# ibrohimmn1994/GPU-implementation-of-signle-and-block-Lanczos

Measured on AMD Instinct MI355X. Metric: block-Lanczos iters/sec + SpMM achieved HBM GB/s vs peak, n=10M nnz=1e8 b=16, higher is better.
Workload: dtype f64; 1 GPU; C3 block Lanczos b=16 fp64, banded-random symmetric CSR n=10000000 per GPU, nnz~10/row, halfwidth 4096; config=C3, n_total=10000000, n_per_gpu=10000000, nnz_per_gpu=100000182, b=16, parallelism=single

## Files before the change

### gpu-implementation-of-signle-and-block-lanczos_amd/__init__.py

```python
from __future__ import annotations

import ctypes
import os
from dataclasses import dataclass
from typing import NamedTuple, Optional

import numpy as np

PKG_DIR = os.path.dirname(os.path.abspath(__file__))
LIB_DIR = os.path.join(PKG_DIR, "lib")
HIP_LIB = os.environ.get("LZ_HIP_LIB") or os.path.join(LIB_DIR, "liblz_hip.so")
HOST_LIB = os.path.join(LIB_DIR, "liblz_host.so")

LZ_F64, LZ_F32 = 0, 1
LZ_ROW_MAJOR, LZ_COL_MAJOR = 0, 1
(LZ_K_SEG768, LZ_K_SEG1536, LZ_K_SEG1024, LZ_K_FNZ, LZ_K_BUF, LZ_K_LDS, LZ_K_ANY_B, LZ_K_CM_DIRECT,
 LZ_K_SPMV) = range(1, 10)
LZ_K_WIN, LZ_K_YCM, LZ_K_EPI, LZ_K_AX3, LZ_K_DOT = 0x100, 0x200, 0x400, 0x800, 0x1000
LZ_K_AX4 = 0x2000
LZ_K_GRAM16, LZ_K_GRAM32F, LZ_K_GRAM_GEN, LZ_K_TSMM16, LZ_K_TSMM32F, LZ_K_TSMM_GEN = range(1, 7)
LZ_K_PGRAM16, LZ_K_PGRAM_GEN, LZ_K_PAPPLY16, LZ_K_PAPPLY_GEN = range(7, 11)
PANEL_GROUP_16, PANEL_GROUP_GEN = 16, 4
PANEL_MAX_BLOCKS = 64
LZ_K_PCOMP16, LZ_K_PCOMP_GEN = 11, 12
PANEL_MAX_KEEP = 16
TRANSPOSE_SHORT, TRANSPOSE_LDS, TRANSPOSE_SCAN_BLOCK = 16, 4096, 2048
CG_THREADS, CG_ROWS_128, CG_GRID_CAP, CG_CHECK_EVERY = 256, 32, 2048, 8
CG_MET, CG_SPENT, CG_NOT_PD = 0, 1, 2
BCG_THREADS, BCG_ROWS_16, BCG_ROWS_32, BCG_ROWS_GEN, BCG_GRID_CAP, BCG_MAX_B = 256, 64, 128, 16, 1024, 32
LZ_K_BCG16, LZ_K_BCG32F, LZ_K_BCG_GEN = 13, 14, 15
BCG_NONE, BCG_CONVERGED, BCG_SPENT, BCG_RANK, BCG_NOT_PD = 0, 1, 2, 3, 4


def bcg_guard(b: int, eps: float) -> float:
    return max(1e-10, 64.0 * b * eps)


# ... 7 lines not shown

_hip = None
_host = None

HIP_SYMBOLS = [
    ("lz_init", _c_int, [_c_int, ctypes.POINTER(_c_vp)]),
    ("lz_finalize", _c_int, [_c_vp]),
    ("lz_set_stream", _c_int, [_c_vp, _c_vp]),
    ("lz_set_final_state", _c_int, [_c_vp, _c_int]),
    ("lz_last_error", ctypes.c_char_p, []),
    ("lz_version", ctypes.c_char_p, []),
    ("lz_device_ok", _c_int, [_c_int]),
    ("lz_device_error", _c_int, [_c_vp, ctypes.POINTER(_c_int)]),
    ("lz_debug_poison_lds", _c_int, [_c_vp, ctypes.c_uint32]),
    ("lz_debug_set_device_error", _c_int, [_c_vp, _c_int]),
    ("lz_debug_fail_next_setup", _c_int, [_c_vp, _c_int]),
    ("lz_prof_enable", _c_int, [_c_vp, _c_int]),
    ("lz_prof_enable_mask", _c_int, [_c_vp, ctypes.c_uint]),
    ("lz_prof_read", _c_int, [_c_vp, _c_int, ctypes.POINTER(_c_dbl), ctypes.POINTER(_c_int)]),
    ("lz_csr_spmm", _c_int, [_c_vp, _c_i64, _c_i64, _c_i64, _c_vp, _c_vp, _c_vp, _c_int, _c_int,
                             _c_vp, _c_i64, _c_int, _c_vp, _c_i64]),
    ("lz_to_row_major", _c_int, [_c_vp, _c_i64, _c_int, _c_int, _c_vp, _c_i64, _c_vp]),
    ("lz_to_col_major", _c_int, [_c_vp, _c_i64, _c_int, _c_int, _c_vp, _c_vp, _c_i64]),
    ("lz_csr_spmv", _c_int, [_c_vp, _c_i64, _c_i64, _c_i64, _c_vp, _c_vp, _c_vp, _c_int, _c_vp, _c_vp]),
    ("lz_gram", _c_int, [_c_vp, _c_i64, _c_int, _c_int, _c_vp, _c_i64, _c_vp]),
    ("lz_sym_cross_gram", _c_int, [_c_vp, _c_i64, _c_int, _c_int, _c_vp, _c_vp, _c_i64, _c_vp]),
    ("lz_tsmm", _c_int, [_c_vp, _c_i64, _c_int, _c_int, _c_dbl, _c_dbl, _c_vp, _c_vp, _c_vp, _c_i64]),
    ("lz_sqrtm_pair", _c_int, [_c_vp, _c_int, _c_int, _c_vp, _c_vp, _c_vp, _c_vp]),
    ("lz_copy_row", _c_int, [_c_vp, _c_int, _c_int, _c_vp, _c_i64, _c_int, _c_i64, _c_vp, _c_i64]),
    ("lz_block_lanczos", _c_int, [_c_vp, _c_i64, _c_i64, _c_vp, _c_vp, _c_vp, _c_int, _c_int, _c_int,
                                  _c_i64, _c_vp, _c_vp, _c_vp, _c_vp, _c_vp, _c_vp, _c_vp]),
    ("lz_block_lanczos_unfused", _c_int, [_c_vp, _c_i64, _c_i64, _c_vp, _c_vp, _c_vp, _c_int, _c_int,
                                          _c_int, _c_i64, _c_vp, _c_vp, _c_vp, _c_vp, _c_vp, _c_vp, _c_vp]),
    ("lz_panel_gram", _c_int, [_c_vp, _c_i64, _c_int, _c_int, _c_int, _c_vp, _c_i64, _c_vp, _c_vp]),
    ("lz_panel_apply", _c_int, [_c_vp, _c_i64, _c_int, _c_int, _c_int, _c_dbl, _c_dbl, _c_vp, _c_i64, _c_vp, _c_vp]),
    ("lz_block_lanczos_reorth", _c_int, [_c_vp, _c_i64, _c_i64, _c_vp, _c_vp, _c_vp, _c_int, _c_int, _c_int,
                                         _c_i64, _c_vp, _c_vp, _c_vp, _c_vp, _c_vp, _c_i64, _c_vp, _c_int]),
    ("lz_panel_compress", _c_int, [_c_vp, _c_i64, _c_int, _c_int, _c_int, _c_int, _c_vp, _c_i64, _c_vp]),
    ("lz_block_lanczos_reorth_resume", _c_int, [_c_vp, _c_i64, _c_i64, _c_vp, _c_vp, _c_vp, _c_int, _c_int, _c_int,
                                                _c_int, _c_i64, _c_vp, _c_vp, _c_vp, _c_vp, _c_vp, _c_i64, _c_vp,
                                                _c_int]),
    ("lz_csr_spmm_axpby", _c_int, [_c_vp, _c_i64, _c_i64, _c_vp, _c_vp, _c_vp, _c_int, _c_int, _c_dbl, _c_vp,
                                   _c_dbl, _c_dbl, _c_vp, _c_vp]),
    ("lz_cheb_apply", _c_int, [_c_vp, _c_i64, _c_i64, _c_vp, _c_vp, _c_vp, _c_int, _c_int, _c_vp, _c_vp, _c_vp,
                               _c_vp]),
    ("lz_col_dots", _c_int, [_c_vp, _c_i64, _c_int, _c_int, _c_vp, _c_vp, _c_vp]),
    ("lz_csr_spmm_axpby_dots", _c_int, [_c_vp, _c_i64, _c_i64, _c_vp, _c_vp, _c_vp, _c_int, _c_int, _c_dbl, _c_vp,
                                        _c_dbl, _c_dbl, _c_vp, _c_vp, _c_vp]),
    ("lz_cheb_moments", _c_int, [_c_vp, _c_i64, _c_i64, _c_vp, _c_vp, _c_vp, _c_int, _c_int, _c_dbl, _c_dbl, _c_int,
                                 _c_vp, _c_vp, _c_vp]),
    ("lz_cg_update", _c_int, [_c_vp, _c_i64, _c_int, _c_int, _c_vp, _c_vp, _c_vp, _c_vp, _c_vp, _c_vp, _c_vp]),
    ("lz_cg_solve", _c_int, [_c_vp, _c_i64, _c_i64, _c_vp, _c_vp, _c_vp, _c_int, _c_int, _c_dbl, _c_vp, _c_vp, _c_vp,
                             _c_vp, _c_vp, _c_vp, _c_vp, _c_vp, _c_vp]),
    ("lz_bcg_update", _c_int, [_c_vp, _c_i64, _c_int, _c_int, _c_vp, _c_vp, _c_vp, _c_vp, _c_vp, _c_vp, _c_vp]),
    ("lz_bcg_direction", _c_int, [_c_vp, _c_i64, _c_int, _c_int, _c_vp, _c_vp, _c_vp, _c_vp]),
    ("lz_bcg_solve", _c_int, [_c_vp, _c_i64, _c_i64, _c_vp, _c_vp, _c_vp, _c_int, _c_int, _c_dbl, _c_vp, _c_vp, _c_vp,
                              _c_vp, _c_vp, _c_vp, _c_vp, _c_vp, _c_vp]),
    ("lz_block_lanczos_reorth_cheb", _c_int, [_c_vp, _c_i64, _c_i64, _c_vp, _c_vp, _c_vp, _c_int, _c_int, _c_int,
                                              _c_i64, _c_vp, _c_vp, _c_vp, _c_vp, _c_vp, _c_i64, _c_vp, _c_int,
                                              _c_vp, _c_vp]),
    ("lz_block_lanczos_reorth_resume_cheb", _c_int, [_c_vp, _c_i64, _c_i64, _c_vp, _c_vp, _c_vp, _c_int, _c_int,
                                                     _c_int, _c_int, _c_i64, _c_vp, _c_vp, _c_vp, _c_vp, _c_vp,
                                                     _c_i64, _c_vp, _c_int, _c_vp, _c_vp]),
    ("lz_csr_spmm_axpby4", _c_int, [_c_vp, _c_i64, _c_i64, _c_vp, _c_vp, _c_vp, _c_int, _c_int, _c_dbl, _c_vp,
                                    _c_dbl, _c_dbl, _c_vp, _c_dbl, _c_vp, _c_vp]),
    ("lz_cheb_series_apply", _c_int, [_c_vp, _c_i64, _c_i64, _c_vp, _c_vp, _c_vp, _c_int, _c_int, _c_int, _c_dbl,
# ... 493 lines not shown
        raise LanczosError("bad CSR file")
    rp = np.empty(n.value + 1, np.int64)
    col = np.empty(nnz.value, np.int32)
    val = np.empty(nnz.value, np.float64 if dt.value == 0 else np.float32)
    if L.lzh_csr_read(path.encode(), _p(rp), _p(col), _p(val)):
        raise LanczosError("CSR read failed")
    return CsrHost(n.value, rp, col, val)


def _torch():
    import torch
    return torch


def _ld(t) -> int:
    if t.shape[1] > 1 and t.stride(1) != 1:
        raise LanczosError("inner dimension must be contiguous")
    return t.stride(0) if t.shape[0] > 1 else t.shape[1]


def _ptr(t) -> Optional[int]:
    return None if t is None else t.data_ptr()


def _dt(t) -> int:
    torch = _torch()
    if t.dtype == torch.float64:
        return LZ_F64
    if t.dtype == torch.float32:
        return LZ_F32
    raise LanczosError(f"unsupported dtype {t.dtype}")


@dataclass
class CsrDevice:
    n: int
    n_cols: int
    row_ptr: "object"
    col: "object"
    val: "object"

    @property
    def nnz(self) -> int:
        return int(self.col.numel())

    @property
    def dtype(self) -> int:
        return _dt(self.val)

    @staticmethod
    def from_host(A: CsrHost, device="cuda", n_cols: Optional[int] = None) -> "CsrDevice":
        torch = _torch()
        return CsrDevice(A.n, A.n if n_cols is None else n_cols,
                         torch.from_numpy(A.row_ptr).to(device),
                         torch.from_numpy(A.col).to(device),
                         torch.from_numpy(A.val).to(device))

    def transpose(self, handle: "Handle") -> "CsrDevice":
        torch = _torch()
        dev = self.val.device
        t_rp = torch.empty(self.n_cols + 1, dtype=torch.int64, device=dev)
        t_col = torch.empty(self.nnz, dtype=torch.int32, device=dev)
        t_val = torch.empty(self.nnz, dtype=self.val.dtype, device=dev)
        _check(handle.L.lz_csr_transpose(handle.ptr, self.n, self.n_cols, self.nnz, _ptr(self.row_ptr), _ptr(self.col),
                                         _ptr(self.val), self.dtype, _ptr(t_rp), _ptr(t_col), _ptr(t_val)),
               "lz_csr_transpose")
        return CsrDevice(self.n_cols, self.n, t_rp, t_col, t_val)


class _ReorthOp(NamedTuple):
    name: str
    head: tuple
    tail: tuple
    filt: object


def _f64(t) -> np.ndarray:
# ... 407 lines not shown
        n, b = W.shape
        _check(self.L.lz_gram(self.ptr, n, b, _dt(W), _ptr(W), W.stride(0), _ptr(R)), "lz_gram")
        return R

    def mm_tt2(self, W, Q, R):
        n, b = W.shape
        if Q.shape != W.shape or (n > 1 and Q.stride(0) != W.stride(0)):
            raise LanczosError("mm_tt2: W and Q must have the same shape and row stride (one ld for both)")
        _check(self.L.lz_sym_cross_gram(self.ptr, n, b, _dt(W), _ptr(W), _ptr(Q), W.stride(0), _ptr(R)),
               "lz_sym_cross_gram")
        return R

    def mm_ts(self, beta: float, alpha: float, Q, S, W):
        n, b = Q.shape
        if W.shape != Q.shape or (n > 1 and Q.stride(0) != W.stride(0)):
            raise LanczosError("mm_ts: Q and W must have the same shape and row stride (one ld for both)")
        _check(self.L.lz_tsmm(self.ptr, n, b, _dt(Q), beta, alpha, _ptr(Q), _ptr(S), _ptr(W), W.stride(0)),
               "lz_tsmm")
        return W

    def sqrtm(self, G, beta, beta_inv, eigval=None):
        b = G.shape[0]
        _check(self.L.lz_sqrtm_pair(self.ptr, b, _dt(G), _ptr(G), _ptr(beta), _ptr(beta_inv), _ptr(eigval)),
               "lz_sqrtm_pair")

    def copy_row_to_vector(self, lc: int, start: int, Q, q, layout: int = LZ_ROW_MAJOR):
        b = Q.shape[1] if layout == LZ_ROW_MAJOR else Q.shape[0]
        _check(self.L.lz_copy_row(self.ptr, b, _dt(Q), _ptr(Q), Q.stride(0), layout, lc, _ptr(q), start),
               "lz_copy_row")

    def block_lanczos_blas(self, A: CsrDevice, B, m: int, lc: int, q, alpha, beta, Q0, Q1, W,
                           fused: bool = True):
        n, b = B.shape
        fn = self.L.lz_block_lanczos if fused else self.L.lz_block_lanczos_unfused
        _check(fn(self.ptr, n, A.nnz, _ptr(A.row_ptr), _ptr(A.col), _ptr(A.val), A.dtype, b, m, lc,
                  _ptr(B), _ptr(q), _ptr(alpha), _ptr(beta), _ptr(Q0), _ptr(Q1), _ptr(W)),
               "lz_block_lanczos")

    @staticmethod
    def _panel(V, vstride: int, n: int, b: int, k: int):
        if V.dim() != 1 or not V.is_contiguous() or V.numel() < (k - 1) * vstride + n * b:
            raise LanczosError("a basis panel is a flat contiguous tensor of at least (k-1)*vstride + n*b elements")

    def panel_gram(self, V, vstride: int, k: int, W, C):
        n, b = W.shape
        self._panel(V, vstride, n, b, max(k, 1))
        if not W.is_contiguous() or not C.is_contiguous() or C.numel() < k * b * b or C.dtype != W.dtype \
                or V.dtype != W.dtype:
            raise LanczosError("panel_gram: W (n, b) and C (k, b, b) contiguous, one dtype")
        _check(self.L.lz_panel_gram(self.ptr, n, b, k, _dt(W), _ptr(V), vstride, _ptr(W), _ptr(C)), "lz_panel_gram")
        return C

    def panel_apply(self, beta: float, alpha: float, V, vstride: int, k: int, S, W):
        n, b = W.shape
        self._panel(V, vstride, n, b, max(k, 1))
        if not W.is_contiguous() or not S.is_contiguous() or S.numel() < k * b * b or S.dtype != W.dtype \
                or V.dtype != W.dtype:
            raise LanczosError("panel_apply: W (n, b) and S (k, b, b) contiguous, one dtype")
        _check(self.L.lz_panel_apply(self.ptr, n, b, k, _dt(W), beta, alpha, _ptr(V), vstride, _ptr(S), _ptr(W)),
               "lz_panel_apply")
        return W

    def block_lanczos_reorth(self, A: CsrDevice, B, m: int, lc: int, q, alpha, beta, V, vstride: int, W,
                             passes: int = 2, filt=None, work=None, normal=None, series=None):
        n, b = B.shape
        self._panel(V, vstride, n, b, max(m, 1))
        op = self._reorth_op("block_lanczos_reorth", A, n, b, W, filt, work, normal, series)
        _check(getattr(self.L, op.name)(self.ptr, *op.head, b, m, lc, _ptr(B), _ptr(q), _ptr(alpha), _ptr(beta),
                                        _ptr(V), vstride, _ptr(W), passes, *op.tail), op.name)

# ... 464 lines not shown
```

### gpu-implementation-of-signle-and-block-lanczos_amd/csrc/lz_api.hip

```cpp
#include <cmath>
#include <cstdarg>
#include <cstdlib>
#include <cstring>
#include <algorithm>
#include <utility>
#include <vector>

#include <type_traits>
#include "lz_comm.hpp"
#include "lz_common.hpp"
#include "lz_internal.hpp"
#include "lz_kernels.hpp"

namespace lz {

static thread_local char g_err[1024] = "";

int prof_begin(lz_handle *h, int cls)
{
    if (!h->prof || !((h->prof_mask >> cls) & 1u) || h->ev_used + 2 > h->ev_cap) return -1;
    const int idx = h->ev_used;
    if (hipEventRecord(h->ev_pool[idx], h->stream) != hipSuccess) return -1;
    h->ev_class[idx / 2] = cls;
    h->ev_used += 2;
// ... 1561 lines not shown
                             int64_t lc, const void *B, void *q, void *alpha, void *beta, void *Q0,
                             void *Q1, void *W)
{
    LZ_HANDLE_CHECK(h);
    LZ_TRY(block_args(n, nnz, rp, col, val, b, m, lc, B, q, alpha, beta, Q0, Q1, W));
    return by_dtype(dtype, [&](auto t) {
        using T = decltype(t);
        return block_lanczos_unfused<T>(h, n, nnz, rp, col, (const T *)val, b, m, lc, (const T *)B, (T *)q,
                                        (T *)alpha, (T *)beta, (T *)Q0, (T *)Q1, (T *)W);
    });
}

int lz_block_lanczos(lz_handle *h, int64_t n, int64_t nnz, const int64_t *rp, const int32_t *col,
                     const void *val, lz_dtype dtype, int b, int m, int64_t lc, const void *B,
                     void *q, void *alpha, void *beta, void *Q0, void *Q1, void *W)
{
    LZ_HANDLE_CHECK(h);
    LZ_TRY(block_args(n, nnz, rp, col, val, b, m, lc, B, q, alpha, beta, Q0, Q1, W));
    return by_dtype(dtype, [&](auto t) -> int {
        using T = decltype(t);
        const T *v = (const T *)val, *Bt = (const T *)B;
        T *qt = (T *)q, *at = (T *)alpha, *bt = (T *)beta, *q0 = (T *)Q0, *q1 = (T *)Q1, *w = (T *)W;
        if constexpr (std::is_same<T, double>::value) {
            if (b == 16) {
                LZ_TRY(solve_begin(h));
                LZ_TRY(block_lanczos_fused16(h, n, nnz, rp, col, v, m, lc, Bt, qt, at, bt, q0, q1, w));
                return solve_status(h);
            }
        }
        return block_lanczos_sep<T>(h, n, nnz, rp, col, v, b, m, lc, Bt, qt, at, bt, q0, q1, w);
    });
}

static int panel_args(int64_t n, int b, int k, lz_dtype dtype, const void *V, int64_t vstride)
{
    LZ_ARG_CHECK(dtype == LZ_F64 || dtype == LZ_F32, "dtype");
    LZ_ARG_CHECK(n >= 1, "n >= 1");
    LZ_ARG_CHECK(b >= 1 && b <= 32, "a basis panel supports 1 <= b <= 32");
    LZ_ARG_CHECK(k >= 1 && k <= kPanelMaxK, "a basis panel holds 1 <= k <= 64 blocks");
    LZ_ARG_CHECK(V != nullptr, "V is NULL");
    LZ_ARG_CHECK(vstride >= n * b, "vstride >= n*b");
    const int64_t per16 = dtype == LZ_F64 ? 2 : 4;
    LZ_ARG_CHECK(vstride % per16 == 0 && reinterpret_cast<uintptr_t>(V) % 16 == 0,
                 "V and vstride must be multiples of 16 bytes");
    return LZ_OK;
}

int lz_panel_gram(lz_handle *h, int64_t n, int b, int k, lz_dtype dtype, const void *V, int64_t vstride,
                  const void *W, void *C)
{
    LZ_HANDLE_CHECK(h);
    LZ_TRY(panel_args(n, b, k, dtype, V, vstride));
    LZ_ARG_CHECK(W && C, "W/C NULL");
    return by_dtype(dtype, [&](auto t) {
        using T = decltype(t);
        return panel_gram<T>(h, n, b, k, (const T *)V, vstride, (const T *)W, (T *)C);
    });
}

int lz_panel_apply(lz_handle *h, int64_t n, int b, int k, lz_dtype dtype, double beta, double alpha, const void *V,
                   int64_t vstride, const void *S, void *W)
{
    LZ_HANDLE_CHECK(h);
    LZ_TRY(panel_args(n, b, k, dtype, V, vstride));
    LZ_ARG_CHECK(S && W, "S/W NULL");
    {
// ... 794 lines not shown
```

### gpu-implementation-of-signle-and-block-lanczos_amd/csrc/lz_common.hpp

```cpp
#pragma once
#include <hip/hip_runtime.h>

#include <cstdint>
#include <cstdio>
#include <string>

#include "lz_hip.h"

namespace lz {

class Comm;

void set_error(const char *fmt, ...);

#define LZ_HIP_TRY(expr)                                                          \
    do {                                                                          \
        hipError_t e_ = (expr);                                                   \
        if (e_ != hipSuccess) {                                                   \
            ::lz::set_error("%s:%d %s -> %s", __FILE__, __LINE__, #expr,          \
                            hipGetErrorString(e_));                               \
            return LZ_E_HIP;                                                      \
        }                                                                         \
    } while (0)

// ... 24 lines not shown
constexpr int kWave = 64;
constexpr int kMaxPartials = 2048;
constexpr int kMaxB = 64;
constexpr int kMaxSolveB = 32;
constexpr size_t kScratchDoubles = 8 * kMaxB * kMaxB;
constexpr size_t kPartials2Doubles = 256 * kMaxB * kMaxB + 4096 * 256;

__host__ __device__ inline int64_t ceil_div(int64_t a, int64_t b) { return (a + b - 1) / b; }

}

struct lz_handle {
    int device = 0;
    hipStream_t stream = nullptr;
    hipStream_t side = nullptr;
    hipEvent_t ev_fork = nullptr, ev_join = nullptr;
    int n_cu = 256;
    int grid_cap = 0;
    double *partials = nullptr;
    size_t partials_cap = 0;
    double *partials2 = nullptr;
    double *scratch = nullptr;
    int *err_flag = nullptr;
    lz::Comm *comm = nullptr;
    int nranks = 1, rank = 0;
    hipStream_t xstream = nullptr;
    hipEvent_t ev_cx = nullptr, ev_xd = nullptr;
    hipEvent_t ev_bd = nullptr;
    int64_t last_split[2] = {-1, -1};
    int last_wf = 0, last_wf_pre = 0;
    int last_kernel[2] = {0, 0};
    int final_state = 1;
    int dbg_setup_fail = 0;
    void *c16buf = nullptr;
    size_t c16_cap = 0;
    int32_t *fnz_colf = nullptr, *fnz_trow = nullptr;
    int64_t fnz_key[4] = {0, 0, 0, 0};
    bool fnz_ok = false;
    void *wf_deps = nullptr;
    int *wf_flags = nullptr;
    size_t wf_deps_cap = 0, wf_flags_cap = 0;
    void *ybuf = nullptr;
    size_t ybuf_cap = 0;
    void *coef = nullptr;
    size_t coef_cap = 0;
    void *tr_ws = nullptr;
    size_t tr_cap = 0;
    void *halo = nullptr;
    uint64_t *pairs = nullptr;
    int *longq = nullptr;
    size_t longq_cap = 0;
    int longq_parity = 0;
    hipStream_t lstream = nullptr;
    hipEvent_t ev_lfork = nullptr, ev_ljoin = nullptr;
    hipStream_t pf_sg = nullptr, pf_sp = nullptr;
    hipEvent_t ev_pff = nullptr, ev_pfg = nullptr, ev_pfp = nullptr;
    int *pf_ctl = nullptr;
    int pf_key = -1;
    int pf_band = 0;
    int64_t pf_band_key[3] = {0, 0, -1};
    size_t pairs_cap = 0;
    void *cm_buf = nullptr;
    size_t cm_cap = 0;
    double *dots_ws = nullptr;
    size_t dots_cap = 0;
    void *cg_ws = nullptr;
// ... 82 lines not shown
```

### gpu-implementation-of-signle-and-block-lanczos_amd/csrc/lz_internal.hpp

```cpp
#pragma once
#include "lz_common.hpp"

namespace lz {

template <typename T>
int spmm_rm(lz_handle *h, int64_t n, int64_t nnz, const int64_t *rp, const int32_t *col, const T *val, int b,
            const T *X, int64_t ldx, int64_t nx, T *Y, int64_t ldy,
            bool ycm = false);
template <typename T>
struct SpmmTerms {
    T a;
    const T *X;
    T c, d;
    const T *Z;
    T e = T(0);
    const T *U = nullptr;
    bool four = false;
};
template <typename T>
int spmm_terms(lz_handle *h, int64_t n, int64_t nnz, const int64_t *rp, const int32_t *col, const T *val, int b,
               SpmmTerms<T> t, T *Y, double *dots = nullptr, bool fused = true, bool fused_dot = true);
template <typename T>
int spmm_cm(lz_handle *h, int64_t n, int64_t nnz, const int64_t *rp, const int32_t *col, const T *val, int b,
            const T *X, int64_t ldx, int64_t nx, T *Y, int64_t ldy);
// ... 97 lines not shown

struct WfPlan {
    bool ok = false;
    int hback = 0, hfwd = 0;
    int nc = 12, tr = 192;
    int var = 0;
    const int16_t *col16 = nullptr;
    int64_t xoff = 0;
    bool planned = false;
};
bool wf_first_gram(int64_t n, int64_t nnz);
int wf_plan16(lz_handle *h, int64_t n, int64_t nnz, const int64_t *rp, const int32_t *col, WfPlan *pl,
              int64_t nx = -1, int64_t xoff = 0);
int wf_reset16(lz_handle *h, int64_t n, const WfPlan &pl);
int wf_step16(lz_handle *h, int64_t n, const int64_t *rp, const int32_t *col, const int16_t *col16,
              const double *val, const uint64_t *pairs, const WfPlan &pl, const double *Yj, const double *Vprev,
              const double *Vj, double *Vout, const double *binv, const double *P1, const double *P2,
              const double *Vg, double *Yo, int epoch, int *nparts, int64_t nx = -1, int64_t p1a = 0,
              int64_t p1b = -1, double *part = nullptr, const int64_t *q = nullptr, double *Vsave = nullptr,
              bool qo = false);
struct WfSlabs {
    static constexpr int kMax = 6;
    const double *p[kMax] = {};
    int g[kMax] = {};
    int k = 0;
    void add(const double *ptr, int nslab)
    {
        p[k] = ptr;
        g[k] = nslab;
        ++k;
    }
};
int wf_fold16(lz_handle *h, const WfSlabs &sl, double *out);
int alpha_wf16(lz_handle *h, const double *part, int P, const double *binv, const double *P1, double *alpha,
               double *P2, const double *V, int64_t lc, int64_t n, double *qrow);

int fused_e32(lz_handle *h, int64_t n, const float *Y, const float *Wj, const float *Wprev, float *Wn,
              const float *binv, const float *P1, int64_t lc, float *qrow, int *nparts);
int fused_u32(lz_handle *h, int64_t n, float *Wn, const float *Wj, const float *P2, int *nparts);
int fused_el32(lz_handle *h, int64_t n, const float *Wj, const float *U, int *nparts);
int fused_ub32(lz_handle *h, int64_t n, const float *U, const float *Wj, const float *binv, const float *P2,
               float *Wn, int *nparts, float *Qa = nullptr,
               float *Qb = nullptr);
int alpha_b2(lz_handle *h, const double *part, int P, const float *binv, float *alpha, float *P2, const float *Wj,
             int64_t lc, int64_t n, float *qrow);
int m_b2(lz_handle *h, const double *part, int P, const float *binv, float *M);
bool spmm_b2_ok(int64_t n, int64_t nnz, int64_t nx);
int fold_slabs_g(lz_handle *h, const double *part, int64_t P, int bb, int G);
int spmm_rm_b2(lz_handle *h, int64_t n, int64_t nnz, const int64_t *rp, const int32_t *col, const float *val,
               const float *X, int64_t nx, float *Y, const float *Wp, const float *Mm, int plan_slot = -1,
               int *slot_out = nullptr, int cap = 768);
int spmm_b2_stage(lz_handle *h, int64_t n, const int64_t *rp, int *cap);
int spmm_b2_plan(lz_handle *h, int64_t n, const int64_t *rp, int cap, int *slot);
template <typename T>
int fused_e_sep(lz_handle *h, int64_t n, int b, const T *Y, const T *Wj, const T *Wprev, T *Wn, const T *binv,
                const T *P1, int64_t lc, T *qrow, int *nparts);
template <typename T>
int fused_u_sep(lz_handle *h, int64_t n, int b, T *Wn, const T *Wj, const T *P2, int *nparts);
template <typename T>
int fused_u_swap_sep(lz_handle *h, int64_t n, int b, T *Wn, T *Xown, const T *P2, int *nparts);

template <typename T>
int vector_lanczos_dev(lz_handle *h, int64_t n, int64_t nnz, const int64_t *rp, const int32_t *col,
                       const T *val, int m, int64_t lc, const T *b, T *q, T *alpha, T *beta, T *q0,
                       T *q1, T *w);

// ... 2 lines not shown
```

### include/lz_hip.h

```cpp
#ifndef LZ_HIP_H
#define LZ_HIP_H
#include <stddef.h>
#include <stdint.h>

#ifdef __cplusplus
extern "C" {
#endif

typedef enum { LZ_F64 = 0, LZ_F32 = 1 } lz_dtype;
typedef enum { LZ_ROW_MAJOR = 0, LZ_COL_MAJOR = 1 } lz_layout;

enum {
    LZ_OK = 0,
    LZ_E_ARG = -1,
    LZ_E_HIP = -2,
    LZ_E_COMM = -3,
    LZ_E_STATE = -4,
    LZ_E_DEVICE = -5
};

typedef struct lz_handle lz_handle;

int lz_init(int device, lz_handle **h);
int lz_finalize(lz_handle *h);
// ... 13 lines not shown
int lz_prof_enable_mask(lz_handle *h, unsigned class_mask);
int lz_prof_read(lz_handle *h, int kernel_class, double *ms_total, int *count);

int lz_csr_spmm(lz_handle *h, int64_t n_rows, int64_t n_cols, int64_t nnz,
                const int64_t *row_ptr, const int32_t *col, const void *val, lz_dtype dtype,
                int b, const void *X, int64_t ldx, lz_layout layout, void *Y, int64_t ldy);

int lz_to_row_major(lz_handle *h, int64_t rows, int b, lz_dtype dtype, const void *X, int64_t ldx, void *Y);

int lz_to_col_major(lz_handle *h, int64_t rows, int b, lz_dtype dtype, const void *X, void *Y, int64_t ldy);

int lz_csr_spmv(lz_handle *h, int64_t n_rows, int64_t n_cols, int64_t nnz,
                const int64_t *row_ptr, const int32_t *col, const void *val, lz_dtype dtype,
                const void *x, void *y);

int lz_gram(lz_handle *h, int64_t n, int b, lz_dtype dtype, const void *W, int64_t ld, void *R);

int lz_sym_cross_gram(lz_handle *h, int64_t n, int b, lz_dtype dtype, const void *W,
                      const void *Q, int64_t ld, void *R);

int lz_tsmm(lz_handle *h, int64_t n, int b, lz_dtype dtype, double beta, double alpha,
            const void *Q, const void *S, void *W, int64_t ld);

int lz_sqrtm_pair(lz_handle *h, int b, lz_dtype dtype, const void *G, void *beta,
                  void *beta_inv, void *eigval);

int lz_copy_row(lz_handle *h, int b, lz_dtype dtype, const void *Q, int64_t ld, lz_layout layout,
                int64_t lc, void *q, int64_t start);

int lz_block_lanczos(lz_handle *h, int64_t n, int64_t nnz, const int64_t *row_ptr,
                     const int32_t *col, const void *val, lz_dtype dtype, int b, int m,
                     int64_t lc, const void *B, void *q, void *alpha, void *beta, void *Q0,
                     void *Q1, void *W);

int lz_block_lanczos_unfused(lz_handle *h, int64_t n, int64_t nnz, const int64_t *row_ptr,
                             const int32_t *col, const void *val, lz_dtype dtype, int b, int m,
                             int64_t lc, const void *B, void *q, void *alpha, void *beta,
                             void *Q0, void *Q1, void *W);

int lz_panel_gram(lz_handle *h, int64_t n, int b, int k, lz_dtype dtype, const void *V, int64_t vstride,
                  const void *W, void *C);
int lz_panel_apply(lz_handle *h, int64_t n, int b, int k, lz_dtype dtype, double beta, double alpha,
                   const void *V, int64_t vstride, const void *S, void *W);
#define LZ_PANEL_MAX_KEEP 16
int lz_panel_compress(lz_handle *h, int64_t n, int b, int k, int r, lz_dtype dtype, void *V, int64_t vstride,
                      const void *Z);

int lz_block_lanczos_reorth(lz_handle *h, int64_t n, int64_t nnz, const int64_t *row_ptr,
                            const int32_t *col, const void *val, lz_dtype dtype, int b, int m,
                            int64_t lc, const void *B, void *q, void *alpha, void *beta, void *V,
                            int64_t vstride, void *W, int passes);

int lz_block_lanczos_reorth_resume(lz_handle *h, int64_t n, int64_t nnz, const int64_t *row_ptr,
                                   const int32_t *col, const void *val, lz_dtype dtype, int b, int r, int m,
                                   int64_t lc, const void *sigma, void *q, void *alpha, void *beta, void *V,
                                   int64_t vstride, void *W, int passes);

int lz_csr_spmm_axpby(lz_handle *h, int64_t n, int64_t nnz, const int64_t *row_ptr, const int32_t *col,
                      const void *val, lz_dtype dtype, int b, double a, const void *X, double c, double d,
                      const void *Z, void *Y);

typedef struct {
    int degree;
    double lo, hi, ref;
} lz_cheb;
int lz_cheb_apply(lz_handle *h, int64_t n, int64_t nnz, const int64_t *row_ptr, const int32_t *col,
// ... 149 lines not shown
```

### include/lz_methods.hpp

```cpp
#ifndef LZ_METHODS_HPP
#define LZ_METHODS_HPP

#include <hip/hip_runtime.h>

#include <cstdint>
#include <memory>
#include <stdexcept>
#include <string>
#include <type_traits>
#include <utility>
#include <vector>

#include "lz_hip.h"
#include "lz_host.h"

namespace lz {

inline void check(int rc, const char *what)
{
    if (rc != 0) throw std::runtime_error(std::string(what) + ": " + lz_last_error());
}
inline void hip_check(hipError_t e, const char *what)
{
    if (e != hipSuccess) throw std::runtime_error(std::string(what) + ": " + hipGetErrorString(e));
// ... 138 lines not shown

template <typename T>
class Csr_matrix {
public:
    Csr_matrix() = default;
    Csr_matrix(int64_t n_rows, int64_t n_cols, const std::vector<int64_t> &rp, const std::vector<int32_t> &col,
               const std::vector<T> &val)
        : n_(n_rows), nc_(n_cols), nnz_((int64_t)col.size()), rp_(rp.data(), rp.size()),
          col_(col.data(), col.size()), val_(val.data(), val.size())
    {
        if ((int64_t)rp.size() != n_rows + 1 || val.size() != col.size())
            throw std::runtime_error("Csr_matrix: inconsistent sizes");
    }
    static Csr_matrix from_ell(int64_t n, int64_t width, const std::vector<double> &data,
                               const std::vector<uint32_t> &idx, bool keep_zeros = false)
    {
        std::vector<int64_t> rp(n + 1);
        const int64_t nnz = lzh_ell_to_csr_count(n, width, data.data(), idx.data(), keep_zeros, rp.data());
        if (nnz < 0) throw std::runtime_error("lzh_ell_to_csr_count failed");
        std::vector<int32_t> col(nnz);
        std::vector<double> v(nnz);
        check(lzh_ell_to_csr_fill(n, width, data.data(), idx.data(), keep_zeros, rp.data(), col.data(), v.data()),
              "lzh_ell_to_csr_fill");
        std::vector<T> vt(v.begin(), v.end());
        return Csr_matrix(n, n, rp, col, vt);
    }
    int64_t n_rows() const { return n_; }
    int64_t n_cols() const { return nc_; }
    int64_t nnz() const { return nnz_; }
    const int64_t *row_ptr() const { return rp_.data(); }
    const int32_t *col() const { return col_.data(); }
    const T *val() const { return val_.data(); }

private:
    int64_t n_ = 0, nc_ = 0, nnz_ = 0;
    DeviceArray<int64_t> rp_;
    DeviceArray<int32_t> col_;
    DeviceArray<T> val_;
};

template <typename T>
void spmm(const Csr_matrix<T> &A, const Dense_matrix<T> &X, Dense_matrix<T> &Y, Context &ctx = default_context())
{
    if (X.layout() != Y.layout() || X.n_cols() != Y.n_cols() || X.n_rows() != A.n_cols() ||
        Y.n_rows() != A.n_rows())
        throw std::runtime_error("spmm: shape or layout mismatch");
    check(lz_csr_spmm(ctx.get(), A.n_rows(), A.n_cols(), A.nnz(), A.row_ptr(), A.col(), A.val(), dtype_of<T>(),
                      X.n_cols(), X.data(), X.ld(), X.layout(), Y.data(), Y.ld()),
          "spmm");
}

template <typename T>
void spmv(const Csr_matrix<T> &A, const Vector<T> &x, Vector<T> &y, Context &ctx = default_context())
{
    check(lz_csr_spmv(ctx.get(), A.n_rows(), A.n_cols(), A.nnz(), A.row_ptr(), A.col(), A.val(), dtype_of<T>(),
                      x.data(), y.data()),
          "spmv");
}

template <typename T>
const T *row_major_block(const Dense_matrix<T> &B, int64_t n, DeviceArray<T> &tmp, Context &ctx, const char *who)
{
    const int b = B.n_cols();
    if (B.n_rows() < n) throw std::runtime_error(std::string(who) + ": B has fewer rows than A");
    if (B.layout() == LZ_ROW_MAJOR) {
        if (B.ld() != b) throw std::runtime_error(std::string(who) + ": a row-major B needs ld = b");
        return B.data();
    }
    tmp = DeviceArray<T>((size_t)n * b);
    check(lz_to_row_major(ctx.get(), n, b, dtype_of<T>(), B.data(), B.ld(), tmp.data()), who);
    return tmp.data();
// ... 23 lines not shown
                               hipMemcpyDeviceToDevice, ctx.stream()),
              who);
}

template <typename T, typename F>
void with_final_blocks(Dense_matrix<T> &Q0, Dense_matrix<T> &Q1, Dense_matrix<T> &W, int64_t n, int b, unsigned m,
                       Context &ctx, const char *who, F call)
{
    for (Dense_matrix<T> *X : {&Q0, &Q1, &W}) check_workspace(*X, n, b, who);
    if (row_major_dense(Q0) && row_major_dense(Q1) && row_major_dense(W)) {
        call(Q0.data(), Q1.data(), W.data());
        return;
    }
    DeviceArray<T> t0((size_t)n * b), t1((size_t)n * b), t2((size_t)n * b);
    call(t0.data(), t1.data(), t2.data());
    store_block(Q0, t0.data(), n, b, ctx, who);
    if (m >= 2) store_block(Q1, t1.data(), n, b, ctx, who);
    store_block(W, t2.data(), n, b, ctx, who);
    ctx.synchronize();
}

template <typename T>
void block_lanczos_blas(const Csr_matrix<T> &A, const Dense_matrix<T> &B, unsigned m, unsigned lc, Vector<T> &q,
                        Dense_matrix<T> *alpha, Dense_matrix<T> *beta, Dense_matrix<T> &Q0, Dense_matrix<T> &Q1,
                        Dense_matrix<T> &W, Context &ctx, Vector<T> *  = nullptr,
                        unsigned  = 0, unsigned  = 0)
{
    const int b = B.n_cols();
    const int64_t n = A.n_rows(), bb = (int64_t)b * b;
    if (q.size() < (int64_t)m * b) throw std::runtime_error("block_lanczos_blas: q needs m*b entries");
    DeviceArray<T> Bt;
    const T *Bp = row_major_block(B, n, Bt, ctx, "block_lanczos_blas");
    DeviceArray<T> al((size_t)m * bb), be((size_t)(m + 1) * bb);
    with_final_blocks(Q0, Q1, W, n, b, m, ctx, "block_lanczos_blas", [&](T *q0, T *q1, T *w) {
        check(lz_block_lanczos(ctx.get(), n, A.nnz(), A.row_ptr(), A.col(), A.val(), dtype_of<T>(), b, (int)m, lc,
                               Bp, q.data(), al.data(), be.data(), q0, q1, w),
              "block_lanczos_blas");
    });
    for (unsigned j = 0; j < m; ++j)
        hip_check(hipMemcpyAsync(alpha[j].data(), al.data() + j * bb, sizeof(T) * bb, hipMemcpyDeviceToDevice,
                                 ctx.stream()), "alpha copy");
    for (unsigned j = 0; j <= m; ++j)
        hip_check(hipMemcpyAsync(beta[j].data(), be.data() + j * bb, sizeof(T) * bb, hipMemcpyDeviceToDevice,
                                 ctx.stream()), "beta copy");
    ctx.synchronize();
}

template <typename T>
void block_lanczos_blas_reference_order(const Csr_matrix<T> &A, const Dense_matrix<T> &B, unsigned m, unsigned lc,
                                        Vector<T> &q, Dense_matrix<T> *alpha, Dense_matrix<T> *beta,
                                        Dense_matrix<T> &Q0, Dense_matrix<T> &Q1, Dense_matrix<T> &W, Context &ctx)
{
    const int b = B.n_cols();
    const int64_t n = A.n_rows(), bb = (int64_t)b * b;
    DeviceArray<T> Bt;
    const T *Bp = row_major_block(B, n, Bt, ctx, "block_lanczos_blas_reference_order");
    DeviceArray<T> al((size_t)m * bb), be((size_t)(m + 1) * bb);
    with_final_blocks(Q0, Q1, W, n, b, m, ctx, "block_lanczos_blas_reference_order", [&](T *q0, T *q1, T *w) {
        check(lz_block_lanczos_unfused(ctx.get(), n, A.nnz(), A.row_ptr(), A.col(), A.val(), dtype_of<T>(), b,
                                       (int)m, lc, Bp, q.data(), al.data(), be.data(), q0, q1, w),
              "block_lanczos_blas_reference_order");
    });
    for (unsigned j = 0; j < m; ++j)
        hip_check(hipMemcpyAsync(alpha[j].data(), al.data() + j * bb, sizeof(T) * bb, hipMemcpyDeviceToDevice,
                                 ctx.stream()), "alpha copy");
    for (unsigned j = 0; j <= m; ++j)
        hip_check(hipMemcpyAsync(beta[j].data(), be.data() + j * bb, sizeof(T) * bb, hipMemcpyDeviceToDevice,
                                 ctx.stream()), "beta copy");
    ctx.synchronize();
// ... 54 lines not shown
```

Baseline: 570.2 iters/s.

## Cache wavefront SpMM plan per CSR matrix and reuse across block-Lanczos calls

Adds a prepare API that builds the wavefront plan for b=16 fp64 (compressed 16-bit columns, tile dependencies, strip pairs) once and stores it on the CSR object. Later block-Lanczos calls adopt the stored plan instead of re-analysing the matrix structure each solve. The plan is keyed on pointers, sizes, tensor versions and env knobs, and falls back to the normal path when it does not apply. This costs extra device memory and some invalidation complexity. The first call still builds the plan and runs the old path.

Result: no change. 569.7 iters/s (-0.1%).

```diff
diff --git a/gpu-implementation-of-signle-and-block-lanczos_amd/__init__.py b/gpu-implementation-of-signle-and-block-lanczos_amd/__init__.py
--- a/gpu-implementation-of-signle-and-block-lanczos_amd/__init__.py
+++ b/gpu-implementation-of-signle-and-block-lanczos_amd/__init__.py
@@ -2,7 +2,7 @@
 
 import ctypes
 import os
-from dataclasses import dataclass
+from dataclasses import dataclass, field
 from typing import NamedTuple, Optional
 
 import numpy as np
@@ -76,6 +76,12 @@
                                   _c_i64, _c_vp, _c_vp, _c_vp, _c_vp, _c_vp, _c_vp, _c_vp]),
     ("lz_block_lanczos_unfused", _c_int, [_c_vp, _c_i64, _c_i64, _c_vp, _c_vp, _c_vp, _c_int, _c_int,
                                           _c_int, _c_i64, _c_vp, _c_vp, _c_vp, _c_vp, _c_vp, _c_vp, _c_vp]),
+    ("lz_wf_prepare_sizes", _c_int, [_c_i64, _c_i64, ctypes.POINTER(ctypes.c_size_t), ctypes.POINTER(ctypes.c_size_t),
+                                     ctypes.POINTER(ctypes.c_size_t)]),
+    ("lz_wf_prepare", _c_int, [_c_vp, _c_i64, _c_i64, _c_vp, _c_vp, _c_vp, _c_vp, _c_vp, _c_vp]),
+    ("lz_block_lanczos_prepared", _c_int, [_c_vp, _c_i64, _c_i64, _c_vp, _c_vp, _c_vp, _c_int, _c_int, _c_int,
+                                           _c_i64, _c_vp, _c_vp, _c_vp, _c_vp, _c_vp, _c_vp, _c_vp, _c_vp]),
+    ("lz_debug_plan_count", _c_int, [_c_vp, ctypes.POINTER(_c_i64), ctypes.POINTER(_c_i64)]),
     ("lz_panel_gram", _c_int, [_c_vp, _c_i64, _c_int, _c_int, _c_int, _c_vp, _c_i64, _c_vp, _c_vp]),
     ("lz_panel_apply", _c_int, [_c_vp, _c_i64, _c_int, _c_int, _c_int, _c_dbl, _c_dbl, _c_vp, _c_i64, _c_vp, _c_vp]),
     ("lz_block_lanczos_reorth", _c_int, [_c_vp, _c_i64, _c_i64, _c_vp, _c_vp, _c_vp, _c_int, _c_int, _c_int,
@@ -635,6 +641,35 @@
     raise LanczosError(f"unsupported dtype {t.dtype}")
 
 
+LZ_WF_PREPARED_VERSION, LZ_WF_KNOB_LEN = 1, 16
+WF_KNOBS = ("LZ_PASS_WF", "LZ_WF_SHAPE", "LZ_PASS1_C16")
+
+
+class WfPrepared(ctypes.Structure):
+    _fields_ = [("struct_size", _c_u32), ("version", _c_u32), ("n", _c_i64), ("nnz", _c_i64),
+                ("row_ptr", _c_vp), ("col", _c_vp), ("col16", _c_vp), ("deps", _c_vp), ("pairs", _c_vp),
+                ("xoff", _c_i64), ("ok", _c_i32), ("col16_ok", _c_i32), ("var", _c_i32), ("nc", _c_i32),
+                ("tr", _c_i32), ("hback", _c_i32), ("hfwd", _c_i32), ("reserved", _c_i32),
+                ("knobs", (ctypes.c_char * LZ_WF_KNOB_LEN) * len(WF_KNOBS))]
+
+
+def wf_prepare_sizes(n: int, nnz: int):
+    s = [ctypes.c_size_t() for _ in range(3)]
+    _check(hip_lib().lz_wf_prepare_sizes(n, nnz, *(ctypes.byref(x) for x in s)), "lz_wf_prepare_sizes")
+    return tuple(int(x.value) for x in s)
+
+
+class _WfPlan(NamedTuple):
+    handle: "object"
+    row_ptr: "object"
+    col: "object"
+    buffers: tuple
+    desc: WfPrepared
+
+
+_WF_PLANS_KEPT = 2
+
+
 @dataclass
 class CsrDevice:
     n: int
@@ -642,10 +677,36 @@
     row_ptr: "object"
     col: "object"
     val: "object"
+    _plans: dict = field(default_factory=dict, init=False, repr=False, compare=False)
 
     @property
     def nnz(self) -> int:
         return int(self.col.numel())
+
+    def invalidate(self) -> None:
+        self._plans.clear()
+
+    def _plan_key(self, handle: "Handle"):
+        return (id(handle), tuple(os.environ.get(k, "") for k in WF_KNOBS)) + tuple(
+            x for t in (self.row_ptr, self.col) for x in (id(t), t.data_ptr(), t.numel(), t._version))
+
+    def _wf_plan(self, handle: "Handle"):
+        key = self._plan_key(handle)
+        plan = self._plans.get(key)
+        if plan is not None:
+            return plan, False
+        torch = _torch()
+        sizes = wf_prepare_sizes(self.n, self.nnz)
+        bufs = tuple(torch.empty(s, dtype=torch.uint8, device=self.col.device) for s in sizes)
+        desc = WfPrepared()
+        _check(handle.L.lz_wf_prepare(handle.ptr, self.n, self.nnz, _ptr(self.row_ptr), _ptr(self.col),
+                                      *(_ptr(t) for t in bufs), ctypes.byref(desc)), "lz_wf_prepare")
+        if not desc.ok:
+            bufs = ()
+        while len(self._plans) >= _WF_PLANS_KEPT:
+            self._plans.pop(next(iter(self._plans)))
+        plan = self._plans[key] = _WfPlan(handle, self.row_ptr, self.col, bufs, desc)
+        return plan, True
 
     @property
     def dtype(self) -> int:
@@ -1119,10 +1180,21 @@
     def block_lanczos_blas(self, A: CsrDevice, B, m: int, lc: int, q, alpha, beta, Q0, Q1, W,
                            fused: bool = True):
         n, b = B.shape
+        args = (n, A.nnz, _ptr(A.row_ptr), _ptr(A.col), _ptr(A.val), A.dtype, b, m, lc,
+                _ptr(B), _ptr(q), _ptr(alpha), _ptr(beta), _ptr(Q0), _ptr(Q1), _ptr(W))
+        if fused and b == 16 and A.dtype == LZ_F64 and n == A.n and hasattr(self.L, "lz_wf_prepare"):
+            plan, made_now = A._wf_plan(self)
+            if not made_now:
+                _check(self.L.lz_block_lanczos_prepared(self.ptr, *args, ctypes.byref(plan.desc)),
+                       "lz_block_lanczos_prepared")
+                return
         fn = self.L.lz_block_lanczos if fused else self.L.lz_block_lanczos_unfused
-        _check(fn(self.ptr, n, A.nnz, _ptr(A.row_ptr), _ptr(A.col), _ptr(A.val), A.dtype, b, m, lc,
-                  _ptr(B), _ptr(q), _ptr(alpha), _ptr(beta), _ptr(Q0), _ptr(Q1), _ptr(W)),
-               "lz_block_lanczos")
+        _check(fn(self.ptr, *args), "lz_block_lanczos")
+
+    def plan_count(self):
+        made, adopted = _c_i64(), _c_i64()
+        _check(self.L.lz_debug_plan_count(self._h, ctypes.byref(made), ctypes.byref(adopted)), "lz_debug_plan_count")
+        return int(made.value), int(adopted.value)
 
     @staticmethod
     def _panel(V, vstride: int, n: int, b: int, k: int):
diff --git a/gpu-implementation-of-signle-and-block-lanczos_amd/csrc/lz_api.hip b/gpu-implementation-of-signle-and-block-lanczos_amd/csrc/lz_api.hip
--- a/gpu-implementation-of-signle-and-block-lanczos_amd/csrc/lz_api.hip
+++ b/gpu-implementation-of-signle-and-block-lanczos_amd/csrc/lz_api.hip
@@ -1617,6 +1617,32 @@
     });
 }
 
+}
+
+int lz::block_lanczos_wf16_planned(lz_handle *h, int64_t n, int64_t nnz, const int64_t *rp, const int32_t *col,
+                                   const double *val, int m, int64_t lc, const double *B, double *q, double *alpha,
+                                   double *beta, double *Q0, double *Q1, double *W, const WfPlan &wp,
+                                   const void *deps, const uint64_t *pairs)
+{
+    LZ_HANDLE_CHECK(h);
+    LZ_TRY(block_args(n, nnz, rp, col, val, 16, m, lc, B, q, alpha, beta, Q0, Q1, W));
+    LZ_ARG_CHECK(wp.ok && wp.tr > 0 && deps && pairs, "planned solve: a plan that applies");
+    const int64_t T = ceil_div(n, (int64_t)wp.tr);
+    LZ_TRY(grow_ws(h, &h->wf_deps, &h->wf_deps_cap, sizeof(int2) * (size_t)(T + 64)));
+    LZ_TRY(grow_ws(h, &h->wf_flags, &h->wf_flags_cap, sizeof(int) * (size_t)(T + 64)));
+    LZ_TRY(solve_begin(h));
+    LZ_HIP_TRY(hipMemcpyAsync(h->wf_deps, deps, sizeof(int2) * (size_t)T, hipMemcpyDeviceToDevice, h->stream));
+    Pass1Plan pl;
+    pl.pairs = pairs;
+    pl.col16 = wp.col16;
+    int P = -1;
+    if (wp.var != 111) LZ_TRY(gram_partials<double>(h, n, 16, B, B, 16, &P));
+    LZ_TRY(block_lanczos_wf16(h, n, nnz, rp, col, val, m, lc, B, q, alpha, beta, Q0, Q1, W, pl, wp, P));
+    return solve_status(h);
+}
+
+extern "C" {
+
 static int panel_args(int64_t n, int b, int k, lz_dtype dtype, const void *V, int64_t vstride)
 {
     LZ_ARG_CHECK(dtype == LZ_F64 || dtype == LZ_F32, "dtype");
diff --git a/gpu-implementation-of-signle-and-block-lanczos_amd/csrc/lz_common.hpp b/gpu-implementation-of-signle-and-block-lanczos_amd/csrc/lz_common.hpp
--- a/gpu-implementation-of-signle-and-block-lanczos_amd/csrc/lz_common.hpp
+++ b/gpu-implementation-of-signle-and-block-lanczos_amd/csrc/lz_common.hpp
@@ -80,6 +80,7 @@
     int last_kernel[2] = {0, 0};
     int final_state = 1;
     int dbg_setup_fail = 0;
+    int64_t plans_made = 0, plans_adopted = 0;
     void *c16buf = nullptr;
     size_t c16_cap = 0;
     int32_t *fnz_colf = nullptr, *fnz_trow = nullptr;
diff --git a/gpu-implementation-of-signle-and-block-lanczos_amd/csrc/lz_internal.hpp b/gpu-implementation-of-signle-and-block-lanczos_amd/csrc/lz_internal.hpp
--- a/gpu-implementation-of-signle-and-block-lanczos_amd/csrc/lz_internal.hpp
+++ b/gpu-implementation-of-signle-and-block-lanczos_amd/csrc/lz_internal.hpp
@@ -153,6 +153,10 @@
     }
 };
 int wf_fold16(lz_handle *h, const WfSlabs &sl, double *out);
+int block_lanczos_wf16_planned(lz_handle *h, int64_t n, int64_t nnz, const int64_t *rp, const int32_t *col,
+                               const double *val, int m, int64_t lc, const double *B, double *q, double *alpha,
+                               double *beta, double *Q0, double *Q1, double *W, const WfPlan &wp,
+                               const void *deps, const uint64_t *pairs);
 int alpha_wf16(lz_handle *h, const double *part, int P, const double *binv, const double *P1, double *alpha,
                double *P2, const double *V, int64_t lc, int64_t n, double *qrow);
 
diff --git a/gpu-implementation-of-signle-and-block-lanczos_amd/csrc/lz_prepare.hip b/gpu-implementation-of-signle-and-block-lanczos_amd/csrc/lz_prepare.hip
--- /dev/null
+++ b/gpu-implementation-of-signle-and-block-lanczos_amd/csrc/lz_prepare.hip
@@ -0,0 +1,134 @@
+#include <cstdlib>
+#include <cstring>
+
+#include "lz_common.hpp"
+#include "lz_internal.hpp"
+#include "lz_kernels.hpp"
+
+namespace lz {
+
+static const char *const kPlanKnobs[LZ_WF_KNOBS] = {"LZ_PASS_WF", "LZ_WF_SHAPE", "LZ_PASS1_C16"};
+constexpr int64_t kWfMinTileRows = 160;
+
+static bool knob_snapshot(char out[LZ_WF_KNOBS][LZ_WF_KNOB_LEN])
+{
+    std::memset(out, 0, (size_t)LZ_WF_KNOBS * LZ_WF_KNOB_LEN);
+    for (int i = 0; i < LZ_WF_KNOBS; ++i) {
+        const char *e = getenv(kPlanKnobs[i]);
+        if (!e) continue;
+        if (std::strlen(e) >= (size_t)LZ_WF_KNOB_LEN) return false;
+        std::strcpy(out[i], e);
+    }
+    return true;
+}
+
+static bool aligned16(const void *p) { return reinterpret_cast<uintptr_t>(p) % 16 == 0; }
+
+static bool plan_applies(const lz_wf_prepared *p, int64_t n, int64_t nnz, const int64_t *rp, const int32_t *col,
+                         lz_dtype dtype, int b)
+{
+    if (!p || p->struct_size != sizeof(lz_wf_prepared) || p->version != LZ_WF_PREPARED_VERSION) return false;
+    if (b != 16 || dtype != LZ_F64 || !p->ok) return false;
+    if (p->n != n || p->nnz != nnz || p->row_ptr != rp || p->col != col) return false;
+    if (!p->deps || !p->pairs || (p->col16_ok && !p->col16) || p->xoff != 0) return false;
+    if (p->nc < 10 || p->nc > 12 || p->tr != 16 * p->nc || (p->var != 0 && p->var != 111 && p->var != 200) ||
+        p->hback < 0 || p->hfwd < 0)
+        return false;
+    char now[LZ_WF_KNOBS][LZ_WF_KNOB_LEN];
+    return knob_snapshot(now) && std::memcmp(now, p->knobs, sizeof(now)) == 0;
+}
+
+}
+
+using namespace lz;
+
+extern "C" {
+
+int lz_wf_prepare_sizes(int64_t n, int64_t nnz, size_t *col16_bytes, size_t *deps_bytes, size_t *pairs_bytes)
+{
+    LZ_ARG_CHECK(n >= 0 && nnz >= 0 && col16_bytes && deps_bytes && pairs_bytes, "prepare sizes");
+    *col16_bytes = (size_t)nnz * 2 + 16;
+    *deps_bytes = sizeof(int32_t) * 2 * (size_t)(ceil_div(n, kWfMinTileRows) + 64);
+    *pairs_bytes = sizeof(uint64_t) * (size_t)(ceil_div(n, (int64_t)16) + kPairPad);
+    return LZ_OK;
+}
+
+int lz_wf_prepare(lz_handle *h, int64_t n, int64_t nnz, const int64_t *row_ptr, const int32_t *col, void *col16,
+                  void *deps, void *pairs, lz_wf_prepared *out)
+{
+    if (!h) {
+        set_error("handle is NULL");
+        return LZ_E_STATE;
+    }
+    LZ_HIP_TRY(hipSetDevice(h->device));
+    LZ_ARG_CHECK(n >= 1 && nnz >= 0 && row_ptr && col && out, "prepare: n >= 1, nnz >= 0, row_ptr / col / out not NULL");
+    LZ_ARG_CHECK(col16 && deps && pairs && aligned16(col16) && aligned16(deps) && aligned16(pairs),
+                 "prepare: three device buffers on 16 bytes");
+    std::memset(out, 0, sizeof(*out));
+    out->struct_size = (uint32_t)sizeof(*out);
+    out->version = LZ_WF_PREPARED_VERSION;
+    out->n = n;
+    out->nnz = nnz;
+    out->row_ptr = row_ptr;
+    out->col = col;
+    out->col16 = col16;
+    out->deps = deps;
+    out->pairs = pairs;
+    ++h->plans_made;
+    if (!knob_snapshot(out->knobs)) return LZ_OK;
+    WfPlan wp;
+    LZ_TRY(wf_plan16(h, n, nnz, row_ptr, col, &wp));
+    out->var = wp.var;
+    out->nc = wp.nc;
+    out->tr = wp.tr;
+    if (!wp.ok) return LZ_OK;
+    const uint64_t *hp = nullptr;
+    LZ_TRY(strip_pairs(h, n, row_ptr, &hp));
+    const int64_t T = ceil_div(n, (int64_t)wp.tr), ns = ceil_div(n, (int64_t)16) + kPairPad;
+    LZ_HIP_TRY(hipMemcpyAsync(deps, h->wf_deps, sizeof(int32_t) * 2 * (size_t)T, hipMemcpyDeviceToDevice, h->stream));
+    LZ_HIP_TRY(hipMemcpyAsync(pairs, hp, sizeof(uint64_t) * (size_t)ns, hipMemcpyDeviceToDevice, h->stream));
+    if (wp.col16)
+        LZ_HIP_TRY(hipMemcpyAsync(col16, wp.col16, sizeof(int16_t) * (size_t)nnz, hipMemcpyDeviceToDevice, h->stream));
+    LZ_HIP_TRY(hipStreamSynchronize(h->stream));
+    out->hback = wp.hback;
+    out->hfwd = wp.hfwd;
+    out->xoff = wp.xoff;
+    out->col16_ok = wp.col16 ? 1 : 0;
+    out->ok = 1;
+    return LZ_OK;
+}
+
+int lz_block_lanczos_prepared(lz_handle *h, int64_t n, int64_t nnz, const int64_t *row_ptr,
+                              const int32_t *col, const void *val, lz_dtype dtype, int b, int m,
+                              int64_t lc, const void *B, void *q, void *alpha, void *beta, void *Q0,
+                              void *Q1, void *W, const lz_wf_prepared *p)
+{
+    if (!h || !plan_applies(p, n, nnz, row_ptr, col, dtype, b))
+        return lz_block_lanczos(h, n, nnz, row_ptr, col, val, dtype, b, m, lc, B, q, alpha, beta, Q0, Q1, W);
+    WfPlan wp;
+    wp.ok = true;
+    wp.hback = p->hback;
+    wp.hfwd = p->hfwd;
+    wp.nc = p->nc;
+    wp.tr = p->tr;
+    wp.var = p->var;
+    wp.col16 = p->col16_ok ? static_cast<const int16_t *>(p->col16) : nullptr;
+    wp.xoff = 0;
+    wp.planned = false;
+    ++h->plans_adopted;
+    return block_lanczos_wf16_planned(h, n, nnz, row_ptr, col, static_cast<const double *>(val), m, lc,
+                                      static_cast<const double *>(B), static_cast<double *>(q),
+                                      static_cast<double *>(alpha), static_cast<double *>(beta),
+                                      static_cast<double *>(Q0), static_cast<double *>(Q1), static_cast<double *>(W), wp,
+                                      p->deps, static_cast<const uint64_t *>(p->pairs));
+}
+
+int lz_debug_plan_count(lz_handle *h, int64_t *made, int64_t *adopted)
+{
+    LZ_ARG_CHECK(h && made && adopted, "NULL argument");
+    *made = h->plans_made;
+    *adopted = h->plans_adopted;
+    return LZ_OK;
+}
+
+}
diff --git a/include/lz_hip.h b/include/lz_hip.h
--- a/include/lz_hip.h
+++ b/include/lz_hip.h
@@ -69,6 +69,36 @@
                      const int32_t *col, const void *val, lz_dtype dtype, int b, int m,
                      int64_t lc, const void *B, void *q, void *alpha, void *beta, void *Q0,
                      void *Q1, void *W);
+
+#define LZ_WF_PREPARED_VERSION 1
+#define LZ_WF_KNOBS 3
+#define LZ_WF_KNOB_LEN 16
+typedef struct lz_wf_prepared {
+    uint32_t struct_size;
+    uint32_t version;
+    int64_t n, nnz;
+    const int64_t *row_ptr;
+    const int32_t *col;
+    void *col16, *deps, *pairs;
+    int64_t xoff;
+    int32_t ok;
+    int32_t col16_ok;
+    int32_t var, nc, tr, hback, hfwd;
+    int32_t reserved;
+    char knobs[LZ_WF_KNOBS][LZ_WF_KNOB_LEN];
+} lz_wf_prepared;
+
+int lz_wf_prepare_sizes(int64_t n, int64_t nnz, size_t *col16_bytes, size_t *deps_bytes, size_t *pairs_bytes);
+
+int lz_wf_prepare(lz_handle *h, int64_t n, int64_t nnz, const int64_t *row_ptr, const int32_t *col, void *col16,
+                  void *deps, void *pairs, lz_wf_prepared *out);
+
+int lz_block_lanczos_prepared(lz_handle *h, int64_t n, int64_t nnz, const int64_t *row_ptr,
+                              const int32_t *col, const void *val, lz_dtype dtype, int b, int m,
+                              int64_t lc, const void *B, void *q, void *alpha, void *beta, void *Q0,
+                              void *Q1, void *W, const lz_wf_prepared *p);
+
+int lz_debug_plan_count(lz_handle *h, int64_t *made, int64_t *adopted);
 
 int lz_block_lanczos_unfused(lz_handle *h, int64_t n, int64_t nnz, const int64_t *row_ptr,
                              const int32_t *col, const void *val, lz_dtype dtype, int b, int m,
diff --git a/include/lz_methods.hpp b/include/lz_methods.hpp
--- a/include/lz_methods.hpp
+++ b/include/lz_methods.hpp
@@ -194,11 +194,33 @@
     const int32_t *col() const { return col_.data(); }
     const T *val() const { return val_.data(); }
 
+    const lz_wf_prepared *wf_plan(Context &ctx, bool *made_now) const
+    {
+        *made_now = false;
+        if (plan_ && plan_->h == ctx.get()) return &plan_->desc;
+        size_t s16 = 0, sd = 0, sp = 0;
+        check(lz_wf_prepare_sizes(n_, nnz_, &s16, &sd, &sp), "lz_wf_prepare_sizes");
+        std::unique_ptr<Plan> p(new Plan{ctx.get(), DeviceArray<unsigned char>(s16), DeviceArray<unsigned char>(sd),
+                                         DeviceArray<unsigned char>(sp), lz_wf_prepared{}});
+        check(lz_wf_prepare(ctx.get(), n_, nnz_, rp_.data(), col_.data(), p->col16.data(), p->deps.data(),
+                            p->pairs.data(), &p->desc),
+              "lz_wf_prepare");
+        plan_ = std::move(p);
+        *made_now = true;
+        return &plan_->desc;
+    }
+
 private:
+    struct Plan {
+        lz_handle *h;
+        DeviceArray<unsigned char> col16, deps, pairs;
+        lz_wf_prepared desc;
+    };
     int64_t n_ = 0, nc_ = 0, nnz_ = 0;
     DeviceArray<int64_t> rp_;
     DeviceArray<int32_t> col_;
     DeviceArray<T> val_;
+    mutable std::unique_ptr<Plan> plan_;
 };
 
 template <typename T>
@@ -288,9 +310,15 @@
     DeviceArray<T> Bt;
     const T *Bp = row_major_block(B, n, Bt, ctx, "block_lanczos_blas");
     DeviceArray<T> al((size_t)m * bb), be((size_t)(m + 1) * bb);
+    const lz_wf_prepared *plan = nullptr;
+    if (b == 16 && std::is_same<T, double>::value) {
+        bool made_now = false;
+        plan = A.wf_plan(ctx, &made_now);
+        if (made_now) plan = nullptr;
+    }
     with_final_blocks(Q0, Q1, W, n, b, m, ctx, "block_lanczos_blas", [&](T *q0, T *q1, T *w) {
-        check(lz_block_lanczos(ctx.get(), n, A.nnz(), A.row_ptr(), A.col(), A.val(), dtype_of<T>(), b, (int)m, lc,
-                               Bp, q.data(), al.data(), be.data(), q0, q1, w),
+        check(lz_block_lanczos_prepared(ctx.get(), n, A.nnz(), A.row_ptr(), A.col(), A.val(), dtype_of<T>(), b,
+                                        (int)m, lc, Bp, q.data(), al.data(), be.data(), q0, q1, w, plan),
               "block_lanczos_blas");
     });
     for (unsigned j = 0; j < m; ++j)
```
